# Sur091/GPU-Ray-Tracing

Hardware: AMD Instinct MI355X
Metric: Mrays/s at 1920×1080 (1/2/4/8 GPUs); achieved HBM GB/s vs roofline (higher is better)
Workload: dtype f32; 1 GPU; K3 configs[2]: 1920x1080, 500 spheres, 1 spp, one progressive update per step, max_depth 1; width=1920, height=1080, spheres=500, max_depth=1, parallelism=stripes1, scan=culled, kernel=rt_tpair_kernel<2>, frame_launch=chain

## Files before the change

### gpu-ray-tracing_amd/csrc/rt_abi.cpp

```cpp
#include <hip/hip_runtime_api.h>

#include <algorithm>
#include <cmath>
#include <cstring>
#include <new>
#include <string>
#include <vector>

#include "rt_adaptive.h"
#include "rt_chain_parts.h"
#include "rt_internal.h"
#include "rt_kernels.h"
#include "rt_certain_tiles.h"
#include "rt_occlusion_cull.h"
#include "rt_selftest_roots.h"

namespace {
thread_local std::string g_last_error = "";
}

namespace rti {

rt_status fail(rt_status s, const std::string& msg) {
    g_last_error = msg;
    return s;
}

rt_status hip_fail(hipError_t e, const char* what) {
    return fail(RT_ERR_HIP, std::string(what) + ": " + hipGetErrorString(e));
}

constexpr uint32_t kMaxDim = 1u << 16;

rt_status check_image(uint32_t w, uint32_t h) {
    if (w == 0 || h == 0 || w > kMaxDim || h > kMaxDim)
        return fail(RT_ERR_INVALID_SIZE, "image size out of range (1..65536 per side)");
    return RT_OK;
}
// ... 146 lines not shown
}

rt_status rt_certain_tiles_stats(rt_ctx* ctx, uint64_t out[2]) {
    if (!ctx) return fail(RT_ERR_INVALID_CONTEXT, "ctx is NULL");
    if (!out) return fail(RT_ERR_INVALID_ARGUMENT, "out is NULL");
    out[0] = out[1] = 0;
    if (!ctx->cand || ctx->cand_live == 0 || ctx->scan_mode != RT_SCAN_CULLED) return RT_OK;
    DeviceGuard guard(ctx->device);
    if (!guard.ok) return fail(RT_ERR_INVALID_DEVICE, "hipSetDevice failed");
    std::vector<uint32_t> flags(ctx->cand_live);
    hipError_t e = hipDeviceSynchronize();
    if (e == hipSuccess)
        e = hipMemcpy2D(flags.data(), sizeof(uint32_t),
                        reinterpret_cast<const uint32_t*>(ctx->cand) + 2,
                        rtk::kCandStride * sizeof(float4), sizeof(uint32_t), ctx->cand_live,
                        hipMemcpyDeviceToHost);
    if (e != hipSuccess) return hip_fail(e, "hipMemcpy2D(tile flags)");
    for (uint32_t f : flags) out[0] += f & rtk::kTileCertain;
    const uint64_t tx = ctx->pair_tiles_x;
    if (ctx->pair_gen == ctx->cand_gen && tx * ctx->pair_bands == ctx->cand_live)
        for (uint64_t b = 0; b < ctx->pair_bands; ++b)
            for (uint64_t x = 0; x + 1 < tx; x += 2)
                out[1] += flags[b * tx + x] & flags[b * tx + x + 1] & rtk::kTileCertain;
    return RT_OK;
}

rt_status rt_create(int device, rt_ctx** out_ctx) {
    if (!out_ctx) return fail(RT_ERR_INVALID_ARGUMENT, "out_ctx is NULL");
    *out_ctx = nullptr;
    int n = 0;
    hipError_t e = hipGetDeviceCount(&n);
    if (e != hipSuccess) return hip_fail(e, "hipGetDeviceCount");
    if (device < 0 || device >= n) return fail(RT_ERR_INVALID_DEVICE, "no such HIP device");
    rt_ctx* ctx = new (std::nothrow) rt_ctx();
    if (!ctx) return fail(RT_ERR_NO_MEMORY, "out of host memory");
    ctx->device = device;
    *out_ctx = ctx;
    return RT_OK;
}

rt_status rt_destroy(rt_ctx* ctx) {
    if (!ctx) return fail(RT_ERR_INVALID_CONTEXT, "ctx is NULL");
    rt_status st = RT_OK;
    {
        DeviceGuard guard(ctx->device);
        if (ctx->d_geom || ctx->d_sph || ctx->cand) (void)hipDeviceSynchronize();
// ... 396 lines not shown
```

### gpu-ray-tracing_amd/csrc/rt_context.h

```cpp
#pragma once

#include <hip/hip_runtime_api.h>

#include <vector>

#include "rt_abi.h"

namespace rtc {
struct Chain;
}

struct rt_ctx {
    int device = 0;
    int scan_mode = RT_SCAN_CULLED;
    float4* d_geom = nullptr;
    float4* d_sph = nullptr;
    uint32_t capacity = 0;
    uint32_t count = 0;
    bool valid = false;
    std::vector<rt_sphere> cached;
    uint64_t scene_gen = 0;
    double scene_bound = 0.0;
    bool radii_ok = true;
    bool normal_rn = false;
    uint32_t* d_flag = nullptr;
    float4* d_hint_rs = nullptr;
    void* d_grid = nullptr;
    struct Grid {
        uint32_t nx = 0, nz = 0, nbig = 0, items = 0;
        float x0, z0, s, inv_s, ylo, yhi, cx, cy, cz, reach, m, e;
    } grid;
    float4* cand = nullptr;
    uint32_t* wg_buf = nullptr;
    uint64_t wg_cap = 0;
    uint32_t wg_pix = 0;
    uint32_t wg_parts = 0;
    uint64_t wg_builds = 0;
    uint64_t band_gen = ~0ull, band_seen_gen = ~0ull;
    uint64_t cand_tiles = 0;
    uint64_t cand_live = 0;
    std::vector<unsigned char> cand_key;
    uint64_t cand_gen = 0;
    bool occlusion_cull = true;
    bool certain_tiles = true;
    uint64_t pair_gen = ~0ull;
    uint32_t pair_tiles_x = 0, pair_bands = 0;
    uint32_t* tile_cost = nullptr;
    uint32_t* tile_order = nullptr;
    uint64_t order_tiles = 0;
    uint64_t chain_raster_key[2] = {0, 0};
    uint64_t cost_gen = ~0ull;
    uint32_t cost_frames = 0;
    uint64_t order_gen = ~0ull;
    uint32_t order_frames = 0;
    uint32_t cost_group = 1;
    uint32_t cost_key[6] = {};
    bool cost_key_ok = false;
    uint32_t* d_band_src = nullptr;
    std::vector<uint32_t> band_src;
    int tile_order_mode = RT_TILE_ORDER_AUTO;
    float* d_srgb = nullptr;
    uint32_t* d_hx = nullptr;
    uint32_t hx_len = 0, hy_len = 0;
    struct CountRecord {
        const void* image;
        uint32_t w, h, first, step, bands, n;
    };
// ... 34 lines not shown
```

### gpu-ray-tracing_amd/csrc/rt_kernels.h

```cpp
#pragma once

#include <hip/hip_runtime_api.h>
#include <stdint.h>

#include "rt_abi.h"

namespace rtk {

constexpr uint32_t kMaxFramesPerLaunch = 128;
constexpr uint32_t kLdsMaxRecords = 4096;
constexpr uint32_t kCandStride = 64;
constexpr uint32_t kCandMax = 19;
constexpr uint32_t kCandRecOff = 1;
constexpr uint32_t kCandSphOff = 21;
constexpr uint32_t kCandNone = 0xFFFFFFFFu;
constexpr uint32_t kTileCertain = 1u;
constexpr uint32_t kClassLambertian = 0u, kClassMetal = 1u, kClassDielectric = 2u;
static_assert(kCandRecOff + ((kCandMax + 3u) & ~3u) <= kCandSphOff, "record chunks fit");
static_assert(kCandSphOff + 2u * kCandMax <= kCandStride, "sphere records fit");
#ifndef RT_HINT_FRAMES
#define RT_HINT_FRAMES 64
#endif
constexpr uint32_t kHintFrames = RT_HINT_FRAMES;
constexpr uint32_t kHintEntries = RT_HINT_FRAMES;
// ... 79 lines not shown
}
constexpr bool is_list_kernel(int k) { return k == kTraceList || is_group_kernel(k); }
#ifndef RT_WG_WAVES
#define RT_WG_WAVES 4
#endif
constexpr bool trace_ordered(int k) {
    return k == kTraceListQuad2 || k == kTraceListPair2 ||
           (is_list_kernel(k) && (is_group_kernel(k) || RT_WG_WAVES == 1));
}
constexpr uint64_t kQuadMaxTiles = 6144;
constexpr uint64_t kQuad2MaxTiles = 20000;
constexpr uint32_t hy_offset(uint32_t width) { return (width + 63u) & ~63u; }
constexpr uint32_t pack_bands(uint32_t first, uint32_t step, bool ordered) {
    return first | ((step < 0x7FFFu ? step : 0x7FFFu) << 16) | (ordered ? 1u << 31 : 0u);
}
hipError_t launch_trace(const TraceParams& p, int kernel, hipStream_t stream);
void arm_launch_events(hipEvent_t start, hipEvent_t stop);
uint32_t disarm_launch_events();
hipError_t launch_deinterleave_bands(const float4* gathered, float4* out, uint32_t width,
                                     uint32_t height, const uint32_t* band_src,
                                     hipStream_t stream);
hipError_t launch_init(float4* out, uint64_t texels, hipStream_t stream);
hipError_t launch_candidates(const TraceParams& p, float4* cand, bool occlusion, bool certain,
                             hipStream_t stream);
hipError_t launch_wg_order(const float4* cand, uint32_t tiles_x, uint32_t bands, uint32_t pix,
                           uint32_t* wg_cost, uint32_t* wg_order, hipStream_t stream,
                           uint32_t parts);
inline void part_range(uint32_t n, uint32_t parts, uint32_t k, uint32_t& first, uint32_t& len) {
    first = k * (n / parts) + (k < n % parts ? k : n % parts);
    len = n / parts + (k < n % parts ? 1u : 0u);
}
uint32_t single_wg_tiles(uint32_t pix);
uint32_t single_pix();
constexpr int kChainPix1 = 0, kChainPix1Reset = 1, kChainPix = 2, kChainPixReset = 3,
              kChainGo = 4, kChainDone = 5, kChainKernels = 6;
constexpr uint32_t kHiddenArgsBytes = 256;
hipError_t chain_load_kernels();
const char* chain_kernel_symbol(int which);
uint32_t chain_args(const TraceParams& p, int kernel, const uint32_t* abort, unsigned char* out,
                    uint32_t cap, uint32_t grid[2], uint32_t* group_threads, int* which);
hipError_t launch_deinterleave(const float4* gathered, float4* out, uint32_t width,
                               uint32_t height, uint32_t nranks, uint32_t max_local_rows,
                               hipStream_t stream);
hipError_t launch_present(const float4* in, uchar4* out, uint64_t texels,
                          const float* srgb_t, hipStream_t stream);
struct AovParams {
    uint32_t* id;
// ... 52 lines not shown
```

### gpu-ray-tracing_amd/csrc/rt_kernels.hip

```cpp
#include <hip/hip_ext.h>
#include <hip/hip_runtime.h>

#include "rt_device.h"
#include "rt_kernels.h"

#include <cstddef>
#include <cstring>

#if defined(__HIP_DEVICE_COMPILE__) && !defined(__gfx950__)
#error "rt_kernels.hip targets gfx950 only (cache-policy bits of the sc1 hand-offs)"
#endif

namespace rtk {

using namespace rtd;

#ifndef RT_WAVE_TRACE
#define RT_WAVE_TRACE 0
#endif
#if RT_WAVE_TRACE
constexpr uint32_t kTraceWaves = 1u << 18;
__device__ unsigned long long g_wave_t[kTraceWaves][2];
__device__ unsigned g_wave_id[kTraceWaves][2];
__device__ __forceinline__ void wave_trace(int end) {
// ... 1653 lines not shown
constexpr uint32_t kCandBY = RT_CAND_BY;
static_assert(kCandBX * kCandBY <= 64, "one lane per tile");
constexpr uint32_t kCandGroup = 8;
constexpr uint32_t kCandStage = 64 * kCandGroup;
__global__ __launch_bounds__(64) void rt_candidates_kernel(const TraceParams p,
                                                           float4* __restrict__ cand,
                                                           const uint32_t occl) {
    __shared__ float4 s_rec[kCandStage];
    __shared__ float4 s_sph[2 * kCandStage];
    __shared__ uint32_t s_idx[kCandStage];
    __shared__ float4 s_own[kCandMax][64];
    __shared__ float s_lo[kCandMax][64];
    const float4* __restrict__ geom = p.geom;
    const float4* __restrict__ gsph = p.sph;
    const uint32_t count = p.count;
    const uint32_t lane = threadIdx.x;
    const uint32_t tiles_x = (p.width + 7u) >> 3;
    const uint32_t tx0 = blockIdx.x * kCandBX, lb0 = blockIdx.y * kCandBY;
    const uint32_t tx1 = min(tx0 + kCandBX, tiles_x);
    const uint32_t lb1 = min(lb0 + kCandBY, p.local_bands);
    const auto row0 = [&](uint32_t lb) {
        return (float)((p.band_first + lb * p.band_step) * RT_STRIPE_ROWS);
    };
    Cone kb;
    const bool in_blk = footprint_cone(p, (float)(tx0 * 8u), (float)(tx1 * 8u), row0(lb0),
                                    row0(lb1 - 1u) + 8.0f, kb);
    const uint32_t tx = tx0 + lane % kCandBX, lb = lb0 + lane / kCandBX;
    const bool mine = tx < tx1 && lb < lb1;
    Cone k;
    const bool ok = mine && footprint_cone(p, (float)(tx * 8u), (float)(tx * 8u + 8u), row0(lb),
                                           row0(lb) + 8.0f, k);
    const uint32_t tile = lb * tiles_x + tx;
    const uint32_t K = min(p.cand_k, kCandMax);
    float4* const own = cand + (size_t)tile * kCandStride;
    float4* const rec = own + kCandRecOff;
    float4* const sph = own + kCandSphOff;
    uint32_t n = 0;
    for (uint32_t gbase = 0; gbase < count; gbase += kCandStage) {
        float4 gv[kCandGroup];
#pragma unroll
        for (uint32_t b = 0; b < kCandGroup; ++b) {
            const uint32_t i = gbase + b * 64u + lane;
            gv[b] = geom[i < count ? i : 0u];
        }
        uint32_t m = 0;
#pragma unroll
        for (uint32_t b = 0; b < kCandGroup; ++b) {
            const uint32_t i = gbase + b * 64u + lane;
            const bool keep = i < count && (!in_blk || !cone_misses(kb, gv[b]));
            const unsigned long long mask = rt_ballot(keep);
            if (keep) {
                const uint32_t pos = m + __builtin_amdgcn_mbcnt_hi(
                    (uint32_t)(mask >> 32), __builtin_amdgcn_mbcnt_lo((uint32_t)mask, 0u));
                s_rec[pos] = gv[b];
                s_idx[pos] = i;
            }
            m += (uint32_t)__builtin_popcountll(mask);
        }
        __syncthreads();
        for (uint32_t j = lane; j < m; j += 64u) {
            const uint32_t i = s_idx[j];
            s_sph[2u * j] = gsph[2u * i];
            s_sph[2u * j + 1u] = gsph[2u * i + 1u];
        }
        __syncthreads();
        for (uint32_t j = 0; j < m; ++j) {
            const float4 gj = s_rec[j];
            if (ok && !cone_misses(k, gj)) {
                if (n < K) {
                    rec[n] = gj;
                    s_own[n][lane] = gj;
                    sph[2u * n] = s_sph[2u * j];
                    sph[2u * n + 1u] = s_sph[2u * j + 1u];
                }
                ++n;
            }
        }
        __syncthreads();
    }
    if (!mine) return;
    uint32_t removed = 0;
    bool front_one = false;
    if ((occl & 1u) && ok && n <= K && n >= 2u) {
        const Lens lens = bundle_lens(p, k);
        float t_occ = __builtin_inff();
        uint32_t j_occ = kCandNone;
        for (uint32_t j = 0; j < n; ++j) {
            const float4 gj = s_own[j][lane];
            const OccBounds b = occ_bounds(k, lens, gj);
            s_lo[j][lane] = b.lo;
            if (b.covers && b.hi < t_occ) {
                t_occ = b.hi;
                j_occ = j;
                front_one = certainly_front(b, gj);
            }
        }
        if (j_occ != kCandNone) {
            uint32_t m = 0;
            for (uint32_t j = 0; j < n; ++j) {
                if (j != j_occ && s_lo[j][lane] > t_occ) continue;
                if (m != j) {
                    rec[m] = s_own[j][lane];
                    sph[2u * m] = sph[2u * j];
                    sph[2u * m + 1u] = sph[2u * j + 1u];
                }
                ++m;
            }
            removed = n - m;
            n = m;
        }
    } else if (occl == 3u && ok && n == 1u && n <= K) {
        const float4 g = s_own[0][lane];
        front_one = certainly_front(occ_bounds(k, bundle_lens(p, k), g), g);
    }
    uint32_t flags = 0;
    if ((occl & 2u) && ok && n <= K && n == 1u && front_one) {
        const float radius = sph[0].w, matw = sph[1].w;
        if (radius > 0.0f && __builtin_isfinite(radius))
            flags = kTileCertain | material_class(matw) << 1;
    }
    const uint32_t c = ok && n <= K ? n : kCandNone;
    if (c != kCandNone)
        for (uint32_t q = n; q < ((n + 3u) & ~3u); ++q)
            rec[q] = make_float4(0.0f, 0.0f, 0.0f, 0.0f);
    own[0] = make_float4(__uint_as_float(c), __uint_as_float(removed), __uint_as_float(flags),
                         0.0f);
}

__global__ __launch_bounds__(256) void rt_init_kernel(float4* __restrict__ out, uint64_t n) {
    const float4 z = make_float4(0.0f, 0.0f, 0.0f, 0.0f);
    for (uint64_t i = (uint64_t)blockIdx.x * blockDim.x + threadIdx.x; i < n;
         i += (uint64_t)gridDim.x * blockDim.x)
        out[i] = z;
}

__global__ __launch_bounds__(256) void rt_deinterleave_kernel(const float4* __restrict__ g,
// ... 350 lines not shown
    grid[1] = g.y;
    *group_threads = 64u * kSingleWg;
    *which = (one ? kChainPix1 : kChainPix) + (p.reset_first ? 1 : 0);
    return total;
}

hipError_t launch_trace(const TraceParams& p, int kernel, hipStream_t stream) {
    if (kernel == kTraceSingle) return launch_single<(int)kSinglePix>(p, stream);
    if (kernel == kTraceSingleOne) return launch_single<1>(p, stream);
    if (kernel == kTraceCulled)
        return launch_trace_as<kTraceCulled>(p, (size_t)p.lds_records * sizeof(float4), stream);
    if (kernel == kTraceList) return launch_trace_as<kTraceList>(p, 0, stream);
    if (kernel == kTraceListPair)
        return launch_trace_as<kTraceListPair>(p, group_lds_bytes<kTraceListPair>(), stream);
    if (kernel == kTraceBounce) return launch_bounce(p, stream);
    if (kernel == kTraceListQuad)
        return launch_trace_as<kTraceListQuad>(p, group_lds_bytes<kTraceListQuad>(), stream);
    if (kernel == kTraceListQuad2) return launch_tpair<4>(p, stream);
    if (kernel == kTraceListPair2) return launch_tpair<2>(p, stream);
    return launch_trace_as<kTraceExhaustive>(p, 0, stream);
}

hipError_t launch_candidates(const TraceParams& p, float4* cand, bool occlusion, bool certain,
                             hipStream_t stream) {
    const uint32_t tiles_x = (p.width + 7u) >> 3;
    const dim3 grid((tiles_x + kCandBX - 1u) / kCandBX,
                    (p.local_bands + kCandBY - 1u) / kCandBY);
    if (grid.x == 0 || grid.y == 0) return hipSuccess;
    hipLaunchKernelGGL(rt_candidates_kernel, grid, dim3(64), 0, stream, p, cand,
                       occlusion ? (certain ? 3u : 1u) : 0u);
    return hipGetLastError();
}

uint32_t single_wg_tiles(uint32_t pix) { return kSingleWg * pix; }
uint32_t single_pix() { return kSinglePix; }

hipError_t launch_wg_order(const float4* cand, uint32_t tiles_x, uint32_t bands, uint32_t pix,
                           uint32_t* wg_cost, uint32_t* wg_order, hipStream_t stream,
                           uint32_t parts) {
    const uint32_t per = kSingleWg * pix;
    const uint32_t cols = (tiles_x + per - 1u) / per;
    const uint32_t units = cols * bands;
    if (units == 0) return hipSuccess;
    hipLaunchKernelGGL(rt_wg_cost_kernel, dim3((units + 255u) / 256u), dim3(256), 0, stream, cand,
                       tiles_x, cols, per, units, wg_cost);
    hipError_t e = hipGetLastError();
    if (e != hipSuccess) return e;
    return launch_tile_order(wg_cost, wg_order, units, cols, stream, parts);
}

hipError_t launch_init(float4* out, uint64_t texels, hipStream_t stream) {
    if (texels == 0) return hipSuccess;
    uint64_t blocks = (texels + 255u) / 256u;
// ... 101 lines not shown
```

### gpu-ray-tracing_amd/csrc/rt_occlusion.h

```cpp
#pragma once

#include "rt_trace_device.h"

namespace rtk {

__device__ __forceinline__ v3 cross3(v3 a, v3 b) {
    return mk(a.y * b.z - a.z * b.y, a.z * b.x - a.x * b.z, a.x * b.y - a.y * b.x);
}
__device__ __forceinline__ float l1(v3 v) { return fabsf(v.x) + fabsf(v.y) + fabsf(v.z); }

struct Lens {
    v3 ctr;
    float rl;
};
__device__ __forceinline__ Lens bundle_lens(const TraceParams& p, const Cone& k) {
    Lens b;
    b.ctr = mk(p.center[0], p.center[1], p.center[2]);
    float rl = 0.0f;
    if (p.defocus_angle > 0.0f) {
        const v3 du = mk(p.ddu[0], p.ddu[1], p.ddu[2]), dv = mk(p.ddv[0], p.ddv[1], p.ddv[2]);
        rl = __builtin_amdgcn_sqrtf(dot(du, du) + dot(dv, dv));
    }
    b.rl = rl * 1.001f + 1e-5f * (l1(k.apex) + l1(b.ctr));
    return b;
}

struct OccBounds {
    float lo, hi;
    bool covers;
    float q2, err;
};
__device__ __forceinline__ OccBounds occ_bounds(const Cone& k, const Lens& b, float4 g) {
    OccBounds r;
    r.lo = -__builtin_inff();
    r.hi = __builtin_inff();
    r.covers = false;
    r.q2 = r.err = 0.0f;
    const v3 C = mk(g.x, g.y, g.z);
    const float R2 = g.w, R = __builtin_amdgcn_sqrtf(g.w);
    const v3 v = sub(C, k.apex);
    const float at = fabsf(dot(v, k.axis)), p = len3(cross3(v, k.axis));
    const float sl = 1e-5f * (at + p + k.r_o) + 1e-6f * (l1(C) + l1(k.apex));
    const float dl_hi = p + at * k.sin_t + k.r_o + sl;
    const float dl_lo = fmaf(p, k.cos_t, -at * k.sin_t) - k.r_o - sl;
    const v3 w = sub(C, b.ctr);
    const float D = len3(w), tc = dot(w, k.axis), pc = len3(cross3(w, k.axis));
    const float sd = 1e-5f * D + 1e-6f * (l1(C) + l1(b.ctr));
    const float s_hi = D + b.rl + sd, s_lo = D - b.rl - sd;
    const bool ahead = tc * k.cos_t - pc * k.sin_t - b.rl - sd > 0.0f && s_lo > R * 1.0001f;
    if (!ahead || !__builtin_isfinite(s_hi + dl_hi + R)) return r;
    const float E = 2e-6f * fmaf(s_hi, s_hi, R2);
    const float q2 = R2 - dl_hi * dl_hi;
    const bool inside = q2 > E;
    const float err = 1e-6f * (s_hi + R) +
                      (inside ? E * __builtin_amdgcn_rsqf(q2) * 1.0001f
                              : __builtin_amdgcn_sqrtf(E) * 1.0001f);
    {
        const float dl = fminf(fmaxf(dl_lo, 0.0f), R);
        const float num = (s_lo - R) * (s_lo + R);
        const float den = __builtin_amdgcn_sqrtf(fmaf(-dl, dl, s_lo * s_lo) * 1.000001f +
                                                 1e-6f * s_lo * s_lo) +
                          __builtin_amdgcn_sqrtf(fmaxf(fmaf(-dl, dl, R2), 0.0f) + 1e-6f * R2);
        r.lo = num / den * 0.9999f - err;
    }
    if (inside) {
        const float num = (s_hi - R) * (s_hi + R);
        const float den =
// ... 24 lines not shown
```

### gpu-ray-tracing_amd/csrc/rt_plan.cpp

```cpp
#include <hip/hip_runtime_api.h>

#include <algorithm>
#include <cmath>
#include <cstdlib>
#include <cstring>
#include <vector>

#include "rt_device.h"
#include "rt_internal.h"
#include "rt_kernels.h"

namespace rti {

int trace_kernel_for(const rt_ctx* ctx, const rtk::TraceParams& p) {
    if (ctx->scan_mode == RT_SCAN_EXHAUSTIVE) return rtk::kTraceExhaustive;
#ifndef RT_FORCE_CULLED_KERNEL
    if (p.depth <= 1u && camera_rays_bounded(ctx, p)) return rtk::kTraceList;
#endif
#ifndef RT_NO_BOUNCE_KERNEL
    if (p.depth >= 2u) return rtk::kTraceBounce;
#endif
    return rtk::kTraceCulled;
}

// ... 27 lines not shown
                                    (tpair && tiles <= rtk::kQuad2MaxTiles)));
    return quad ? (tpair ? rtk::kTraceListQuad2 : rtk::kTraceListQuad)
                : (tpair ? rtk::kTraceListPair2 : rtk::kTraceListPair);
}

UnitGrid frame_group_units(int kernel, uint32_t w, uint32_t bands) {
    const uint32_t group =
        kernel == rtk::kTraceListQuad2 || kernel == rtk::kTraceListPair2 ? 2u : 1u;
    const uint32_t units_x = (((w + 7u) >> 3) + group - 1u) / group;
    return {group, units_x, (uint64_t)units_x * bands};
}

void free_candidates(rt_ctx* ctx) {
    (void)hipFree(ctx->cand);
    ctx->cand = nullptr;
    ctx->cand_tiles = 0;
    ctx->cand_live = 0;
    ctx->cand_key.clear();
}

static rt_status ensure_candidates(rt_ctx* ctx, rtk::TraceParams& p, hipStream_t stream) {
    struct Key {
        float center[3], vul[3], pdu[3], pdv[3], ddu[3], ddv[3], defocus;
        uint32_t w, h, first, step, bands, occlusion, certain;
        uint64_t scene;
    } key;
    std::memset(&key, 0, sizeof(key));
    std::memcpy(key.center, p.center, sizeof(key.center));
    std::memcpy(key.vul, p.vul, sizeof(key.vul));
    std::memcpy(key.pdu, p.pdu, sizeof(key.pdu));
    std::memcpy(key.pdv, p.pdv, sizeof(key.pdv));
    std::memcpy(key.ddu, p.ddu, sizeof(key.ddu));
    std::memcpy(key.ddv, p.ddv, sizeof(key.ddv));
    key.defocus = p.defocus_angle;
    key.w = p.width;
    key.h = p.height;
    key.first = p.band_first;
    key.step = p.band_step;
    key.bands = p.local_bands;
    key.scene = ctx->scene_gen;
    const bool occlusion = ctx->occlusion_cull && ctx->scene_bound <= 0x1p40 &&
                           camera_rays_bounded(ctx, p);
    key.occlusion = occlusion ? 1u : 0u;
    const bool certain = occlusion && ctx->certain_tiles;
    key.certain = certain ? 1u : 0u;
    const unsigned char* kb = reinterpret_cast<const unsigned char*>(&key);
    const uint64_t tiles = launch_tiles(p.width, p.local_bands);
    p.cand_k = rtk::kCandMax;
    if (ctx->cand_key.size() != sizeof(key) ||
        std::memcmp(ctx->cand_key.data(), kb, sizeof(key)) != 0) {
        if (tiles > ctx->cand_tiles) {
            if (ctx->cand_tiles) {
                hipError_t e = hipStreamSynchronize(stream);
                if (e != hipSuccess) return hip_fail(e, "hipStreamSynchronize");
            }
            free_candidates(ctx);
            hipError_t e = hipMalloc(&ctx->cand, tiles * rtk::kCandStride * sizeof(float4));
            if (e != hipSuccess) {
                free_candidates(ctx);
                return hip_fail(e, "hipMalloc(candidate lists)");
            }
            ctx->cand_tiles = tiles;
        }
        hipError_t e = rtk::launch_candidates(p, ctx->cand, occlusion, certain, stream);
        if (e != hipSuccess) return hip_fail(e, "rt_candidates_kernel launch");
        ctx->cand_key.assign(kb, kb + sizeof(key));
        ctx->cand_gen++;
        ctx->cand_live = tiles;
    }
    p.cand = ctx->cand;
    return RT_OK;
}

rt_status ensure_order_buffers(rt_ctx* ctx, uint64_t tiles, hipStream_t stream) {
    if (tiles <= ctx->order_tiles) return RT_OK;
    if (ctx->order_tiles) {
        hipError_t e = hipStreamSynchronize(stream);
        if (e != hipSuccess) return hip_fail(e, "hipStreamSynchronize");
    }
    (void)hipFree(ctx->tile_cost);
    (void)hipFree(ctx->tile_order);
    ctx->tile_cost = ctx->tile_order = nullptr;
    ctx->order_tiles = 0;
    ctx->cost_gen = ctx->order_gen = ~0ull;
    ctx->chain_raster_key[0] = 0;
    hipError_t e = hipMalloc(&ctx->tile_cost, tiles * sizeof(uint32_t));
    if (e == hipSuccess) e = hipMalloc(&ctx->tile_order, 3 * tiles * sizeof(uint32_t));
// ... 415 lines not shown
```

### gpu-ray-tracing_amd/csrc/rt_trace_device.h

```cpp
#pragma once

#include <hip/hip_runtime.h>

#include "rt_device.h"
#include "rt_kernels.h"

#include <cstddef>
#include <cstring>

#if defined(__HIP_DEVICE_COMPILE__) && !defined(__gfx950__)
#error "rt_trace_device.h targets gfx950 only"
#endif

#ifndef WAVE_TRACE
#define WAVE_TRACE(e) ((void)0)
#endif
#ifndef BCOUNT
#define BCOUNT(k) ((void)0)
#endif
#ifndef SST_V
#define SST_V(k, dep) ((void)0)
#endif
#ifndef SST_S
#define SST_S(k, dep) ((void)0)
// ... 440 lines not shown
    const uint32_t lane = threadIdx.x & 63u;
    const float a = dot(d, d);
    float tmax = t_seed;
    int idx = -1;
    for (uint32_t base = 0; base < count; base += 64u) {
        const float4 g = recs[base + lane];
        const bool keep = (base + lane < count) && !cone_misses(k, g);
        unsigned long long mask = rt_ballot(keep);
        while (mask) {
            const int j = __builtin_ctzll(mask);
            mask &= mask - 1ull;
            const float4 gs = recs[base + (uint32_t)j];
            float h;
            const float disc = discriminant(gs, o, d, a, h);
            consider(disc, h, a, base + (uint32_t)j, tmax, idx);
        }
        if (kOcc && rt_ballot(live && idx < 0) == 0ull) break;
    }
    return Hit{idx, tmax};
}

__device__ __forceinline__ float len3(v3 v) { return __builtin_amdgcn_sqrtf(dot(v, v)); }

__device__ __forceinline__ bool footprint_cone(const TraceParams& p, float x0, float x1,
                                               float y0, float y1, Cone& k) {
    const v3 vul = mk(p.vul[0], p.vul[1], p.vul[2]), pdu = mk(p.pdu[0], p.pdu[1], p.pdu[2]),
             pdv = mk(p.pdv[0], p.pdv[1], p.pdv[2]);
    const v3 ctr = mk(p.center[0], p.center[1], p.center[2]);
    const v3 pc = fmas(0.5f * (y0 + y1), pdv, fmas(0.5f * (x0 + x1), pdu, vul));
    float rq = 0.0f;
#pragma unroll
    for (int c = 0; c < 4; ++c) {
        const v3 q = fmas(c & 2 ? y1 : y0, pdv, fmas(c & 1 ? x1 : x0, pdu, vul));
        rq = fmaxf(rq, len3(sub(q, pc)));
    }
    float rl = 0.0f;
    if (p.defocus_angle > 0.0f) {
        const v3 du = mk(p.ddu[0], p.ddu[1], p.ddu[2]), dv = mk(p.ddv[0], p.ddv[1], p.ddv[2]);
        rl = __builtin_amdgcn_sqrtf(dot(du, du) + dot(dv, dv));
    }
    const float mag = fabsf(pc.x) + fabsf(pc.y) + fabsf(pc.z) + fabsf(ctr.x) + fabsf(ctr.y) +
                      fabsf(ctr.z);
    rq = rq * 1.001f + 1e-5f * mag;
    rl = rl * 1.001f + 1e-5f * mag;
    const v3 w = sub(pc, ctr);
    const float L = len3(w), delta = rq + rl;
    if (!(L > 4.0f * delta) || !__builtin_isfinite(L + mag)) return false;
    k.axis = mk(w.x / L, w.y / L, w.z / L);
    k.apex = pc;
    k.sin_t = delta / (L - delta) * 1.01f;
    k.cos_t = __builtin_amdgcn_sqrtf(1.0f - k.sin_t * k.sin_t) * 0.999f;
    k.r_o = rq;
    k.d_max = (L + delta) * 1.001f;
    return true;
}

struct Cam {
    v3 center, vul, pdu, pdv, ddu, ddv;
    float defocus_angle;
    float k1s = -0x1.9943f2p-13f, k1c = 0x1.99eb9cp-16f;
};
template <typename P>
__device__ __forceinline__ Cam cam_params(const P& p) {
    Cam cam;
    cam.center = mk(p.center[0], p.center[1], p.center[2]);
    cam.vul = mk(p.vul[0], p.vul[1], p.vul[2]);
    cam.pdu = mk(p.pdu[0], p.pdu[1], p.pdu[2]);
    cam.pdv = mk(p.pdv[0], p.pdv[1], p.pdv[2]);
    cam.ddu = mk(p.ddu[0], p.ddu[1], p.ddu[2]);
    cam.ddv = mk(p.ddv[0], p.ddv[1], p.ddv[2]);
    cam.defocus_angle = p.defocus_angle;
    return cam;
}

template <int kTable>
__device__ __forceinline__ void disk_unit(float sa, float ca, float& ux, float& uy) {
    const float len2 = fmaf(sa, sa, ca * ca);
// ... 273 lines not shown
```

### gpu-ray-tracing_amd/gpu_ray_tracing/_lib.py

```python
from __future__ import annotations

import ctypes
import os
from pathlib import Path

import torch

PKG_ROOT = Path(__file__).resolve().parent.parent
LIB_PATH = PKG_ROOT / "build" / "librt_hip.so"

F = ctypes.c_float
U32 = ctypes.c_uint32


class RtError(RuntimeError):

    def __init__(self, status: int, func: str, message: str):
        super().__init__(f"{func} failed with status {status} ({STATUS_NAMES.get(status, '?')}): "
                         f"{message}")
        self.status = status


STATUS_NAMES = {
    0: "RT_OK",
# ... 102 lines not shown
    "rt_band_costs": (ctypes.c_int, [P, U32, U32, P, P]),
    "rt_partition_bands": (ctypes.c_int, [P, U32, U32, P]),
    "rt_deinterleave_bands": (ctypes.c_int, [P, P, P, U32, U32, U32, P, U32, P]),
    "rt_gather_bands": (ctypes.c_int, [P, P, P, P, P, U32, U32, P, U32, P]),
    "rt_set_launch_timing": (ctypes.c_int, [P, ctypes.c_int]),
    "rt_last_call_kernel_time": (ctypes.c_int, [P, ctypes.POINTER(F), ctypes.POINTER(U32)]),
}

_SIGS_CHAIN_PARTS = {
    "rt_set_chain_parts": (ctypes.c_int, [P, U32]),
    "rt_chain_schedule": (ctypes.c_int, [U32, U32, ctypes.c_int, P, U32, ctypes.POINTER(U32)]),
}

_SIGS_OCCLUSION = {
    "rt_set_occlusion_cull": (ctypes.c_int, [P, ctypes.c_int]),
    "rt_occlusion_cull_stats": (ctypes.c_int, [P, P]),
}

_SIGS_CERTAIN = {
    "rt_set_certain_tiles": (ctypes.c_int, [P, ctypes.c_int]),
    "rt_certain_tiles_stats": (ctypes.c_int, [P, P]),
}

_SIGS_SELFTEST_ROOTS = {
    "rt_selftest_roots": (ctypes.c_int, [P, ctypes.c_uint64, P]),
}
RT_ROOTS_FAMILIES = 2
RT_ROOTS_STRATA = 4

_SIGS_AOV = {
    "rt_trace_aov": (ctypes.c_int, [P, P, U32, U32, P, P, U32, P]),
    "rt_trace_aov_bands": (ctypes.c_int, [P, P, U32, U32, P, P, P, U32, P]),
    "rt_pick": (ctypes.c_int, [P, U32, U32, U32, U32, P, P, U32, P, P]),
}
RT_AOV_MISS = 0xFFFFFFFF
AOV_PLANES = ("sphere_id", "hit", "normal", "material")


class AovPlanesC(ctypes.Structure):
    _fields_ = [("sphere_id", P), ("hit", P), ("normal", P), ("material", P)]


class PickResultC(ctypes.Structure):
    _fields_ = [("sphere_id", U32), ("t", F), ("p", F * 3), ("normal", F * 3),
                ("front_face", U32), ("color", F * 4)]

# ... 170 lines not shown
    _fields_ = [("part", U32), ("first", U32), ("frames", U32)]


class RootsTallyC(ctypes.Structure):
    _fields_ = [("mismatches", ctypes.c_uint64), ("drawn", ctypes.c_uint64),
                ("compared", ctypes.c_uint64), ("rooted", ctypes.c_uint64)]


_lib = None


def lib() -> ctypes.CDLL:
    global _lib
    if _lib is None:
        path = Path(os.environ.get("RT_HIP_LIB", LIB_PATH))
        if not path.exists():
            raise RuntimeError(f"librt_hip.so not found at {path}: build it with "
                               f"`make -C {PKG_ROOT}` (no CPU fallback exists)")
        handle = ctypes.CDLL(str(path))
        for name, (res, args) in {**_SIGS, **_SIGS_CHAIN_PARTS, **_SIGS_SELFTEST_ROOTS,
                                  **_SIGS_AOV, **_SIGS_DENOISE, **_SIGS_REPROJECT,
                                  **_SIGS_VARIANCE, **_SIGS_ADAPTIVE, **_SIGS_CONVERGE,
                                  **_SIGS_PROGRESS, **_SIGS_EDIT, **_SIGS_OCCLUSION,
                                  **_SIGS_MATTE, **_SIGS_QUERY, **_SIGS_CERTAIN}.items():
            if "RT_HIP_LIB" in os.environ and not hasattr(handle, name):
                continue
            fn = getattr(handle, name)
            fn.restype = res
            fn.argtypes = args
        _lib = handle
    return _lib


_fast = False


def fastcall():
    global _fast
    if _fast is False:
        _fast = None
        if "RT_HIP_LIB" not in os.environ:
            import importlib.machinery
            import importlib.util
            import sysconfig
            path = PKG_ROOT / "build" / ("_rt_fastcall" + sysconfig.get_config_var("EXT_SUFFIX"))
            if path.exists():
                lib()
# ... 2 lines not shown
                                                              loader=loader)
                mod = importlib.util.module_from_spec(spec)
                loader.exec_module(mod)
                _fast = mod
    return _fast


def exported_symbols() -> list[str]:
    return list(_SIGS)


def chain_parts_symbols() -> list[str]:
    return list(_SIGS_CHAIN_PARTS)


def occlusion_symbols() -> list[str]:
    return list(_SIGS_OCCLUSION)


def certain_symbols() -> list[str]:
    return list(_SIGS_CERTAIN)


def selftest_roots_symbols() -> list[str]:
    return list(_SIGS_SELFTEST_ROOTS)


def aov_symbols() -> list[str]:
    return list(_SIGS_AOV)


def denoise_symbols() -> list[str]:
    return list(_SIGS_DENOISE)


def reproject_symbols() -> list[str]:
    return list(_SIGS_REPROJECT)


def variance_symbols() -> list[str]:
    return list(_SIGS_VARIANCE)


def adaptive_symbols() -> list[str]:
    return list(_SIGS_ADAPTIVE)

# ... 30 lines not shown
```

### gpu-ray-tracing_amd/gpu_ray_tracing/compute_shader.py

```python
from __future__ import annotations

import ctypes

import numpy as np
import torch

from . import _lib
from .camera import SceneCamera
from .scene import SphereCollection

RT_STRIPE_ROWS = _lib.RT_STRIPE_ROWS
DENOISE_DEFAULTS = {"iterations": 5, "normal_power_log2": 5, "sigma_color": 1.0,
                    "sigma_position": 0.5}


REPROJECT_DEFAULTS = {"max_history": 64, "position_tolerance2": 1e-5, "lambertian_only": True}


GUIDED_DEFAULTS = {"iterations": 5, "normal_power_log2": 5, "sigma_luminance": 1.0,
                   "sigma_position": 0.5, "min_history": 4, "fallback_variance": 1.0}


ADAPTIVE_DEFAULTS = {"min_samples": 16, "abs_tolerance2": 1e-5, "rel_tolerance2": 2.5e-4}

# ... 146 lines not shown
        _lib.call("rt_set_frame_images", self._ctx, {"last_two": 0, "every": 1}[mode])

    def set_tile_order(self, mode: str) -> None:
        _lib.call("rt_set_tile_order", self._ctx, {"auto": 0, "off": 1}[mode])

    def set_update_queues(self, queues: int) -> None:
        _lib.call("rt_set_update_queues", self._ctx, int(queues))

    def set_chain_parts(self, parts: int) -> None:
        _lib.call("rt_set_chain_parts", self._ctx, int(parts))

    def set_occlusion_cull(self, on: bool) -> None:
        _lib.call("rt_set_occlusion_cull", self._ctx, 1 if on else 0)

    def set_certain_tiles(self, on: bool) -> None:
        if hasattr(_lib.lib(), "rt_set_certain_tiles"):
            _lib.call("rt_set_certain_tiles", self._ctx, 1 if on else 0)

    def certain_tiles_stats(self) -> dict:
        out = (ctypes.c_uint64 * 2)()
        if hasattr(_lib.lib(), "rt_certain_tiles_stats"):
            _lib.call("rt_certain_tiles_stats", self._ctx, out)
        return {"certain_tiles": int(out[0]), "certain_pairs": int(out[1])}

    def set_update_submit(self, mode: str) -> None:
        _lib.call("rt_set_update_submit", self._ctx, {"auto": 0, "hip": 1, "aql": 2}[mode])

    def submit_status(self) -> dict:
        avail, give_ups, packets = ctypes.c_int(0), _lib.U32(0), ctypes.c_uint64(0)
        _lib.call("rt_update_submit_status", self._ctx, ctypes.byref(avail),
                  ctypes.byref(give_ups), ctypes.byref(packets))
        why = "" if avail.value else _lib.lib().rt_last_error().decode()
        return {"aql_available": bool(avail.value), "go_give_ups": int(give_ups.value),
                "packets": int(packets.value), "why": why}

    def set_path_compaction(self, mode: str) -> None:
        _lib.call("rt_set_path_compaction", self._ctx,
                  {"auto": 0, "per_wave": 1, "compact": 2, "pair": 3, "split": 4}[mode])

    def set_single_kernel(self, mode: str) -> None:
        _lib.call("rt_set_single_kernel", self._ctx,
                  {"auto": 0, "off": 1, "pair": 2, "one": 3}[mode])

    def frames_per_launch(self, camera) -> int:
        out = _lib.U32(0)
        cam = camera.to_c()
# ... 843 lines not shown
```

Baseline: 211,900 Mrays/s.

## Replace per-tile footprint cone with tighter beam bound for candidate culling

Replaces the cone bounding each tile's ray footprint with a beam model. The beam uses a smaller half-angle, a separate near-side spread term, and a tighter lens radius taken from the largest eigenvalue of the defocus disk. The intent is to cull more spheres from each tile's candidate list and to let occlusion and certain-tile tests succeed more often, so the trace kernel scans fewer spheres per pixel. It also adds a toggle to fall back to the old parent cone and a host API to dump tile lists. Tighter bounds risk false culls if the conservative margins are wrong.

```diff
diff --git a/gpu-ray-tracing_amd/csrc/rt_abi.cpp b/gpu-ray-tracing_amd/csrc/rt_abi.cpp
--- a/gpu-ray-tracing_amd/csrc/rt_abi.cpp
+++ b/gpu-ray-tracing_amd/csrc/rt_abi.cpp
@@ -14,6 +14,7 @@
 #include "rt_certain_tiles.h"
 #include "rt_occlusion_cull.h"
 #include "rt_selftest_roots.h"
+#include "rt_tile_lists.h"
 
 namespace {
 thread_local std::string g_last_error = "";
@@ -206,6 +207,43 @@
         for (uint64_t b = 0; b < ctx->pair_bands; ++b)
             for (uint64_t x = 0; x + 1 < tx; x += 2)
                 out[1] += flags[b * tx + x] & flags[b * tx + x + 1] & rtk::kTileCertain;
+    return RT_OK;
+}
+
+rt_status rt_set_tight_bundle(rt_ctx* ctx, int on) {
+    if (!ctx) return fail(RT_ERR_INVALID_CONTEXT, "ctx is NULL");
+    if (on != 0 && on != 1) return fail(RT_ERR_INVALID_ARGUMENT, "on must be 0 or 1");
+    ctx->tight_bundle = on != 0;
+    return RT_OK;
+}
+
+static_assert(RT_TILE_LIST_MAX == rtk::kCandMax && rtk::kCandRecOff == 1u &&
+                  sizeof(rt_tile_list) == (1u + rtk::kCandMax) * sizeof(float4) &&
+                  RT_TILE_LIST_NONE == rtk::kCandNone && RT_TILE_CERTAIN == rtk::kTileCertain,
+              "rt_tile_list mirrors the candidate block");
+
+rt_status rt_tile_lists(rt_ctx* ctx, rt_tile_list* out, uint64_t capacity, uint64_t* tiles) {
+    if (!ctx) return fail(RT_ERR_INVALID_CONTEXT, "ctx is NULL");
+    if (!tiles) return fail(RT_ERR_INVALID_ARGUMENT, "tiles is NULL");
+    *tiles = 0;
+    if (!ctx->cand || ctx->cand_live == 0 || ctx->scan_mode != RT_SCAN_CULLED) return RT_OK;
+    *tiles = ctx->cand_live;
+    const uint64_t n = std::min<uint64_t>(ctx->cand_live, capacity);
+    if (!out || n == 0) return RT_OK;
+    DeviceGuard guard(ctx->device);
+    if (!guard.ok) return fail(RT_ERR_INVALID_DEVICE, "hipSetDevice failed");
+    hipError_t e = hipDeviceSynchronize();
+    if (e == hipSuccess)
+        e = hipMemcpy2D(out, sizeof(rt_tile_list), ctx->cand, rtk::kCandStride * sizeof(float4),
+                        sizeof(rt_tile_list), n, hipMemcpyDeviceToHost);
+    if (e != hipSuccess) return hip_fail(e, "hipMemcpy2D(tile lists)");
+    for (uint64_t t = 0; t < n; ++t) {
+        rt_tile_list& l = out[t];
+        l.reserved = 0;
+        const uint32_t kept = l.count == RT_TILE_LIST_NONE ? 0u : std::min(l.count, RT_TILE_LIST_MAX);
+        if (kept < RT_TILE_LIST_MAX)
+            std::memset(l.records[kept], 0, (RT_TILE_LIST_MAX - kept) * sizeof(l.records[0]));
+    }
     return RT_OK;
 }
 
diff --git a/gpu-ray-tracing_amd/csrc/rt_context.h b/gpu-ray-tracing_amd/csrc/rt_context.h
--- a/gpu-ray-tracing_amd/csrc/rt_context.h
+++ b/gpu-ray-tracing_amd/csrc/rt_context.h
@@ -43,6 +43,7 @@
     uint64_t cand_gen = 0;
     bool occlusion_cull = true;
     bool certain_tiles = true;
+    bool tight_bundle = true;
     uint64_t pair_gen = ~0ull;
     uint32_t pair_tiles_x = 0, pair_bands = 0;
     uint32_t* tile_cost = nullptr;
diff --git a/gpu-ray-tracing_amd/csrc/rt_kernels.h b/gpu-ray-tracing_amd/csrc/rt_kernels.h
--- a/gpu-ray-tracing_amd/csrc/rt_kernels.h
+++ b/gpu-ray-tracing_amd/csrc/rt_kernels.h
@@ -125,7 +125,7 @@
                                      hipStream_t stream);
 hipError_t launch_init(float4* out, uint64_t texels, hipStream_t stream);
 hipError_t launch_candidates(const TraceParams& p, float4* cand, bool occlusion, bool certain,
-                             hipStream_t stream);
+                             bool tight, hipStream_t stream);
 hipError_t launch_wg_order(const float4* cand, uint32_t tiles_x, uint32_t bands, uint32_t pix,
                            uint32_t* wg_cost, uint32_t* wg_order, hipStream_t stream,
                            uint32_t parts);
diff --git a/gpu-ray-tracing_amd/csrc/rt_kernels.hip b/gpu-ray-tracing_amd/csrc/rt_kernels.hip
--- a/gpu-ray-tracing_amd/csrc/rt_kernels.hip
+++ b/gpu-ray-tracing_amd/csrc/rt_kernels.hip
@@ -1699,14 +1699,15 @@
     const auto row0 = [&](uint32_t lb) {
         return (float)((p.band_first + lb * p.band_step) * RT_STRIPE_ROWS);
     };
-    Cone kb;
-    const bool in_blk = footprint_cone(p, (float)(tx0 * 8u), (float)(tx1 * 8u), row0(lb0),
-                                    row0(lb1 - 1u) + 8.0f, kb);
+    const bool parent = (occl & 4u) != 0u;
+    Beam kb;
+    const bool in_blk = footprint_beam(p, (float)(tx0 * 8u), (float)(tx1 * 8u), row0(lb0),
+                                    row0(lb1 - 1u) + 8.0f, parent, kb);
     const uint32_t tx = tx0 + lane % kCandBX, lb = lb0 + lane / kCandBX;
     const bool mine = tx < tx1 && lb < lb1;
-    Cone k;
-    const bool ok = mine && footprint_cone(p, (float)(tx * 8u), (float)(tx * 8u + 8u), row0(lb),
-                                           row0(lb) + 8.0f, k);
+    Beam k;
+    const bool ok = mine && footprint_beam(p, (float)(tx * 8u), (float)(tx * 8u + 8u), row0(lb),
+                                           row0(lb) + 8.0f, parent, k);
     const uint32_t tile = lb * tiles_x + tx;
     const uint32_t K = min(p.cand_k, kCandMax);
     float4* const own = cand + (size_t)tile * kCandStride;
@@ -1724,7 +1725,7 @@
 #pragma unroll
         for (uint32_t b = 0; b < kCandGroup; ++b) {
             const uint32_t i = gbase + b * 64u + lane;
-            const bool keep = i < count && (!in_blk || !cone_misses(kb, gv[b]));
+            const bool keep = i < count && (!in_blk || !beam_misses(kb, gv[b]));
             const unsigned long long mask = rt_ballot(keep);
             if (keep) {
                 const uint32_t pos = m + __builtin_amdgcn_mbcnt_hi(
@@ -1743,7 +1744,7 @@
         __syncthreads();
         for (uint32_t j = 0; j < m; ++j) {
             const float4 gj = s_rec[j];
-            if (ok && !cone_misses(k, gj)) {
+            if (ok && !beam_misses(k, gj)) {
                 if (n < K) {
                     rec[n] = gj;
                     s_own[n][lane] = gj;
@@ -1759,7 +1760,7 @@
     uint32_t removed = 0;
     bool front_one = false;
     if ((occl & 1u) && ok && n <= K && n >= 2u) {
-        const Lens lens = bundle_lens(p, k);
+        const Lens lens = bundle_lens(p, k, parent);
         float t_occ = __builtin_inff();
         uint32_t j_occ = kCandNone;
         for (uint32_t j = 0; j < n; ++j) {
@@ -1786,9 +1787,9 @@
             removed = n - m;
             n = m;
         }
-    } else if (occl == 3u && ok && n == 1u && n <= K) {
+    } else if ((occl & 3u) == 3u && ok && n == 1u && n <= K) {
         const float4 g = s_own[0][lane];
-        front_one = certainly_front(occ_bounds(k, bundle_lens(p, k), g), g);
+        front_one = certainly_front(occ_bounds(k, bundle_lens(p, k, parent), g), g);
     }
     uint32_t flags = 0;
     if ((occl & 2u) && ok && n <= K && n == 1u && front_one) {
@@ -2185,13 +2186,13 @@
 }
 
 hipError_t launch_candidates(const TraceParams& p, float4* cand, bool occlusion, bool certain,
-                             hipStream_t stream) {
+                             bool tight, hipStream_t stream) {
     const uint32_t tiles_x = (p.width + 7u) >> 3;
     const dim3 grid((tiles_x + kCandBX - 1u) / kCandBX,
                     (p.local_bands + kCandBY - 1u) / kCandBY);
     if (grid.x == 0 || grid.y == 0) return hipSuccess;
     hipLaunchKernelGGL(rt_candidates_kernel, grid, dim3(64), 0, stream, p, cand,
-                       occlusion ? (certain ? 3u : 1u) : 0u);
+                       (occlusion ? (certain ? 3u : 1u) : 0u) | (tight ? 0u : 4u));
     return hipGetLastError();
 }
 
diff --git a/gpu-ray-tracing_amd/csrc/rt_occlusion.h b/gpu-ray-tracing_amd/csrc/rt_occlusion.h
--- a/gpu-ray-tracing_amd/csrc/rt_occlusion.h
+++ b/gpu-ray-tracing_amd/csrc/rt_occlusion.h
@@ -13,14 +13,10 @@
     v3 ctr;
     float rl;
 };
-__device__ __forceinline__ Lens bundle_lens(const TraceParams& p, const Cone& k) {
+__device__ __forceinline__ Lens bundle_lens(const TraceParams& p, const Beam& k, bool parent) {
     Lens b;
     b.ctr = mk(p.center[0], p.center[1], p.center[2]);
-    float rl = 0.0f;
-    if (p.defocus_angle > 0.0f) {
-        const v3 du = mk(p.ddu[0], p.ddu[1], p.ddu[2]), dv = mk(p.ddv[0], p.ddv[1], p.ddv[2]);
-        rl = __builtin_amdgcn_sqrtf(dot(du, du) + dot(dv, dv));
-    }
+    const float rl = lens_radius(p, parent);
     b.rl = rl * 1.001f + 1e-5f * (l1(k.apex) + l1(b.ctr));
     return b;
 }
@@ -30,7 +26,7 @@
     bool covers;
     float q2, err;
 };
-__device__ __forceinline__ OccBounds occ_bounds(const Cone& k, const Lens& b, float4 g) {
+__device__ __forceinline__ OccBounds occ_bounds(const Beam& k, const Lens& b, float4 g) {
     OccBounds r;
     r.lo = -__builtin_inff();
     r.hi = __builtin_inff();
@@ -39,10 +35,11 @@
     const v3 C = mk(g.x, g.y, g.z);
     const float R2 = g.w, R = __builtin_amdgcn_sqrtf(g.w);
     const v3 v = sub(C, k.apex);
-    const float at = fabsf(dot(v, k.axis)), p = len3(cross3(v, k.axis));
+    const float t = dot(v, k.axis), at = fabsf(t), p = len3(cross3(v, k.axis));
+    const float spread = beam_spread(k, t);
     const float sl = 1e-5f * (at + p + k.r_o) + 1e-6f * (l1(C) + l1(k.apex));
-    const float dl_hi = p + at * k.sin_t + k.r_o + sl;
-    const float dl_lo = fmaf(p, k.cos_t, -at * k.sin_t) - k.r_o - sl;
+    const float dl_hi = p + spread + k.r_o + sl;
+    const float dl_lo = fmaf(p, k.cos_t, -spread) - k.r_o - sl;
     const v3 w = sub(C, b.ctr);
     const float D = len3(w), tc = dot(w, k.axis), pc = len3(cross3(w, k.axis));
     const float sd = 1e-5f * D + 1e-6f * (l1(C) + l1(b.ctr));
diff --git a/gpu-ray-tracing_amd/csrc/rt_plan.cpp b/gpu-ray-tracing_amd/csrc/rt_plan.cpp
--- a/gpu-ray-tracing_amd/csrc/rt_plan.cpp
+++ b/gpu-ray-tracing_amd/csrc/rt_plan.cpp
@@ -73,7 +73,7 @@
 static rt_status ensure_candidates(rt_ctx* ctx, rtk::TraceParams& p, hipStream_t stream) {
     struct Key {
         float center[3], vul[3], pdu[3], pdv[3], ddu[3], ddv[3], defocus;
-        uint32_t w, h, first, step, bands, occlusion, certain;
+        uint32_t w, h, first, step, bands, occlusion, certain, tight;
         uint64_t scene;
     } key;
     std::memset(&key, 0, sizeof(key));
@@ -95,6 +95,7 @@
     key.occlusion = occlusion ? 1u : 0u;
     const bool certain = occlusion && ctx->certain_tiles;
     key.certain = certain ? 1u : 0u;
+    key.tight = ctx->tight_bundle ? 1u : 0u;
     const unsigned char* kb = reinterpret_cast<const unsigned char*>(&key);
     const uint64_t tiles = launch_tiles(p.width, p.local_bands);
     p.cand_k = rtk::kCandMax;
@@ -113,7 +114,8 @@
             }
             ctx->cand_tiles = tiles;
         }
-        hipError_t e = rtk::launch_candidates(p, ctx->cand, occlusion, certain, stream);
+        hipError_t e = rtk::launch_candidates(p, ctx->cand, occlusion, certain,
+                                              ctx->tight_bundle, stream);
         if (e != hipSuccess) return hip_fail(e, "rt_candidates_kernel launch");
         ctx->cand_key.assign(kb, kb + sizeof(key));
         ctx->cand_gen++;
diff --git a/gpu-ray-tracing_amd/csrc/rt_trace_device.h b/gpu-ray-tracing_amd/csrc/rt_trace_device.h
--- a/gpu-ray-tracing_amd/csrc/rt_trace_device.h
+++ b/gpu-ray-tracing_amd/csrc/rt_trace_device.h
@@ -486,8 +486,24 @@
 
 __device__ __forceinline__ float len3(v3 v) { return __builtin_amdgcn_sqrtf(dot(v, v)); }
 
-__device__ __forceinline__ bool footprint_cone(const TraceParams& p, float x0, float x1,
-                                               float y0, float y1, Cone& k) {
+__device__ __forceinline__ float lens_radius(const TraceParams& p, bool parent) {
+    if (!(p.defocus_angle > 0.0f)) return 0.0f;
+    const v3 du = mk(p.ddu[0], p.ddu[1], p.ddu[2]), dv = mk(p.ddv[0], p.ddv[1], p.ddv[2]);
+    const float a = dot(du, du), b = dot(dv, dv), c = dot(du, dv);
+    if (parent) return __builtin_amdgcn_sqrtf(a + b);
+    const float h = 0.5f * (a + b), g = 0.5f * (a - b);
+    return __builtin_amdgcn_sqrtf(h + __builtin_amdgcn_sqrtf(fmaf(g, g, c * c))) * 1.0001f;
+}
+
+struct Beam {
+    v3 apex, axis;
+    float cos_t, sin_t;
+    float sin_n;
+    float r_o, d_max;
+};
+
+__device__ __forceinline__ bool footprint_beam(const TraceParams& p, float x0, float x1,
+                                               float y0, float y1, bool parent, Beam& k) {
     const v3 vul = mk(p.vul[0], p.vul[1], p.vul[2]), pdu = mk(p.pdu[0], p.pdu[1], p.pdu[2]),
              pdv = mk(p.pdv[0], p.pdv[1], p.pdv[2]);
     const v3 ctr = mk(p.center[0], p.center[1], p.center[2]);
@@ -498,11 +514,7 @@
         const v3 q = fmas(c & 2 ? y1 : y0, pdv, fmas(c & 1 ? x1 : x0, pdu, vul));
         rq = fmaxf(rq, len3(sub(q, pc)));
     }
-    float rl = 0.0f;
-    if (p.defocus_angle > 0.0f) {
-        const v3 du = mk(p.ddu[0], p.ddu[1], p.ddu[2]), dv = mk(p.ddv[0], p.ddv[1], p.ddv[2]);
-        rl = __builtin_amdgcn_sqrtf(dot(du, du) + dot(dv, dv));
-    }
+    float rl = lens_radius(p, parent);
     const float mag = fabsf(pc.x) + fabsf(pc.y) + fabsf(pc.z) + fabsf(ctr.x) + fabsf(ctr.y) +
                       fabsf(ctr.z);
     rq = rq * 1.001f + 1e-5f * mag;
@@ -512,11 +524,33 @@
     if (!(L > 4.0f * delta) || !__builtin_isfinite(L + mag)) return false;
     k.axis = mk(w.x / L, w.y / L, w.z / L);
     k.apex = pc;
-    k.sin_t = delta / (L - delta) * 1.01f;
+    if (parent) {
+        k.sin_t = delta / (L - delta) * 1.01f;
+        k.sin_n = k.sin_t;
+    } else {
+        k.sin_t = delta / L * 1.01f;
+        const float sn = (rl - rq) / L;
+        k.sin_n = sn * (sn > 0.0f ? 1.01f : 0.99f);
+    }
     k.cos_t = __builtin_amdgcn_sqrtf(1.0f - k.sin_t * k.sin_t) * 0.999f;
     k.r_o = rq;
     k.d_max = (L + delta) * 1.001f;
     return true;
+}
+
+__device__ __forceinline__ float beam_spread(const Beam& k, float t) {
+    return fmaxf(fmaxf(k.sin_t * t, -k.sin_n * t), fmaf(-k.sin_t, t, -2.0f * k.r_o));
+}
+
+__device__ __forceinline__ bool beam_misses(const Beam& k, float4 g) {
+    const v3 v = mk(g.x - k.apex.x, g.y - k.apex.y, g.z - k.apex.z);
+    const float t = dot(v, k.axis);
+    const float p = __builtin_amdgcn_sqrtf(fmaxf(fmaf(-t, t, dot(v, v)), 0.0f));
+    const float at = fabsf(t), R = __builtin_amdgcn_sqrtf(g.w) * 1.0001f;
+    const float mag = at + p + k.r_o;
+    const float lhs = fmaf(p, k.cos_t, -beam_spread(k, t)) - k.r_o - 1e-5f * mag;
+    const float m = 2.5e-3f * (mag + k.d_max + R);
+    return lhs > R && lhs * lhs > fmaf(R, R, m * m) * 1.0001f;
 }
 
 struct Cam {
diff --git a/gpu-ray-tracing_amd/gpu_ray_tracing/_lib.py b/gpu-ray-tracing_amd/gpu_ray_tracing/_lib.py
--- a/gpu-ray-tracing_amd/gpu_ray_tracing/_lib.py
+++ b/gpu-ray-tracing_amd/gpu_ray_tracing/_lib.py
@@ -148,6 +148,20 @@
     "rt_certain_tiles_stats": (ctypes.c_int, [P, P]),
 }
 
+_SIGS_TILE_LISTS = {
+    "rt_tile_lists": (ctypes.c_int, [P, P, ctypes.c_uint64, ctypes.POINTER(ctypes.c_uint64)]),
+    "rt_set_tight_bundle": (ctypes.c_int, [P, ctypes.c_int]),
+}
+RT_TILE_LIST_MAX = 19
+RT_TILE_LIST_NONE = 0xFFFFFFFF
+RT_TILE_CERTAIN = 1
+
+
+class TileListC(ctypes.Structure):
+    _fields_ = [("count", U32), ("removed", U32), ("flags", U32), ("reserved", U32),
+                ("records", (ctypes.c_float * 4) * RT_TILE_LIST_MAX)]
+
+
 _SIGS_SELFTEST_ROOTS = {
     "rt_selftest_roots": (ctypes.c_int, [P, ctypes.c_uint64, P]),
 }
@@ -364,7 +378,8 @@
                                   **_SIGS_AOV, **_SIGS_DENOISE, **_SIGS_REPROJECT,
                                   **_SIGS_VARIANCE, **_SIGS_ADAPTIVE, **_SIGS_CONVERGE,
                                   **_SIGS_PROGRESS, **_SIGS_EDIT, **_SIGS_OCCLUSION,
-                                  **_SIGS_MATTE, **_SIGS_QUERY, **_SIGS_CERTAIN}.items():
+                                  **_SIGS_MATTE, **_SIGS_QUERY, **_SIGS_CERTAIN,
+                                  **_SIGS_TILE_LISTS}.items():
             if "RT_HIP_LIB" in os.environ and not hasattr(handle, name):
                 continue
             fn = getattr(handle, name)
@@ -413,6 +428,10 @@
     return list(_SIGS_CERTAIN)
 
 
+def tile_lists_symbols() -> list[str]:
+    return list(_SIGS_TILE_LISTS)
+
+
 def selftest_roots_symbols() -> list[str]:
     return list(_SIGS_SELFTEST_ROOTS)
 
diff --git a/gpu-ray-tracing_amd/gpu_ray_tracing/compute_shader.py b/gpu-ray-tracing_amd/gpu_ray_tracing/compute_shader.py
--- a/gpu-ray-tracing_amd/gpu_ray_tracing/compute_shader.py
+++ b/gpu-ray-tracing_amd/gpu_ray_tracing/compute_shader.py
@@ -192,6 +192,20 @@
         if hasattr(_lib.lib(), "rt_certain_tiles_stats"):
             _lib.call("rt_certain_tiles_stats", self._ctx, out)
         return {"certain_tiles": int(out[0]), "certain_pairs": int(out[1])}
+
+    def set_tight_bundle(self, on: bool) -> None:
+        if hasattr(_lib.lib(), "rt_set_tight_bundle"):
+            _lib.call("rt_set_tight_bundle", self._ctx, 1 if on else 0)
+
+    def tile_lists(self) -> dict:
+        n = ctypes.c_uint64(0)
+        _lib.call("rt_tile_lists", self._ctx, None, 0, ctypes.byref(n))
+        buf = np.zeros((int(n.value), 4 + 4 * _lib.RT_TILE_LIST_MAX), np.uint32)
+        assert buf.shape[1] * buf.itemsize == ctypes.sizeof(_lib.TileListC)
+        if n.value:
+            _lib.call("rt_tile_lists", self._ctx, buf.ctypes.data, n.value, ctypes.byref(n))
+        return {"count": buf[:, 0].copy(), "removed": buf[:, 1].copy(), "flags": buf[:, 2].copy(),
+                "records": buf[:, 4:].copy().view(np.float32).reshape(-1, _lib.RT_TILE_LIST_MAX, 4)}
 
     def set_update_submit(self, mode: str) -> None:
         _lib.call("rt_set_update_submit", self._ctx, {"auto": 0, "hip": 1, "aql": 2}[mode])
diff --git a/include/rt_tile_lists.h b/include/rt_tile_lists.h
--- /dev/null
+++ b/include/rt_tile_lists.h
@@ -0,0 +1,31 @@
+#ifndef RT_TILE_LISTS_H
+#define RT_TILE_LISTS_H
+
+#include "rt_abi.h"
+
+#ifdef __cplusplus
+extern "C" {
+#endif
+
+#define RT_TILE_LIST_MAX 19u
+#define RT_TILE_LIST_NONE 0xFFFFFFFFu
+#define RT_TILE_CERTAIN 1u
+
+typedef struct rt_tile_list {
+    uint32_t count;
+    uint32_t removed;
+    uint32_t flags;
+    uint32_t reserved;
+    float records[RT_TILE_LIST_MAX][4];
+} rt_tile_list;
+
+RT_API rt_status rt_tile_lists(rt_ctx* ctx, rt_tile_list* out, uint64_t capacity,
+                               uint64_t* tiles);
+
+RT_API rt_status rt_set_tight_bundle(rt_ctx* ctx, int on);
+
+#ifdef __cplusplus
+}
+#endif
+
+#endif
```

Measured after the change: 216,900 Mrays/s (median of 6 runs). 1.02x the previous value.
